# mukteshkrmishra/namazu

Hardware: AMD Instinct MI355X
Metric: schedule decisions/sec + trace-pair edit distances/sec at 1/2/4/8 MI355X (higher is better)
Workload: dtype u64; 1 GPU; configs[1] replayable seed sweep; seeds_per_gpu=1048576, events=4096, max_interval_ns=100000000, topk=64, pipeline_streams=3, parallelism=seed-range x1

## Files before the change

### include/nmz_gpu.h

```cpp
#ifndef NMZ_GPU_H
#define NMZ_GPU_H

#include <stddef.h>
#include <stdint.h>

#ifdef __cplusplus
extern "C" {
#endif

#define NMZ_ABI_VERSION 1

#define NMZ_OK 0
#define NMZ_EINVAL (-1)
#define NMZ_EHIP (-2)
#define NMZ_ENOMEM (-3)
#define NMZ_ERANGE (-4)
#define NMZ_EAGAIN (-5)

#define NMZ_EV_PRIORITIZED 0x01u
#define NMZ_EV_FAULTABLE 0x02u

#define NMZ_STAT_RNG_OVERFLOW 0x01u

#define NMZ_NONE 0xffffffffu
// ... 61 lines not shown
                         uint64_t n_seeds, const uint32_t *hint_off, const uint8_t *hint_bytes,
                         uint32_t n_events, int64_t max_interval_ns, nmz_sched_stats *stats,
                         int64_t *delays, uint64_t n_dump_seeds, uint32_t k,
                         nmz_topk_entry *topk);

typedef struct nmz_replayable_plan nmz_replayable_plan;
int nmz_replayable_plan_create(nmz_ctx *ctx, const uint32_t *hint_off, const uint8_t *hint_bytes,
                               uint32_t n_events, int64_t max_interval_ns,
                               uint64_t max_seeds, nmz_replayable_plan **out);
int nmz_replayable_plan_create_async(nmz_ctx *ctx, const uint32_t *hint_off, const uint8_t *hint_bytes,
                                     uint32_t n_events, int64_t max_interval_ns, uint64_t max_seeds,
                                     nmz_replayable_plan **out);
typedef struct nmz_replayable_seeds nmz_replayable_seeds;
int nmz_replayable_seeds_create(nmz_ctx *ctx, const uint32_t *d_seed_off, const uint8_t *d_seed_bytes,
                                uint64_t n_seeds, uint64_t dec_lo, nmz_replayable_seeds **out);
int nmz_replayable_seeds_destroy(nmz_replayable_seeds *seeds);
int nmz_replayable_sweep_seeds_topk_dev(nmz_replayable_plan *plan, const nmz_replayable_seeds *seeds, uint64_t seed0,
                                        uint32_t k, nmz_sched_stats *d_stats, nmz_topk_entry *d_topk, void *stream);
int nmz_replayable_sweep_traces(nmz_ctx *ctx, uint32_t n_traces, const uint32_t *const *hint_off,
                                const uint8_t *const *hint_bytes, const uint32_t *n_events, int64_t max_interval_ns,
                                uint64_t seed_lo, uint64_t n_seeds, uint32_t k, nmz_topk_entry *topk);
int nmz_replayable_plan_destroy(nmz_replayable_plan *plan);
int nmz_replayable_plan_kernel(const nmz_replayable_plan *plan);
int nmz_replayable_sweep_dev(nmz_replayable_plan *plan, const uint32_t *d_seed_off,
                             const uint8_t *d_seed_bytes, uint64_t n_seeds,
                             nmz_sched_stats *d_stats, void *stream);
int nmz_replayable_sweep_topk_dev(nmz_replayable_plan *plan, const uint32_t *d_seed_off,
                                  const uint8_t *d_seed_bytes, uint64_t n_seeds, uint64_t seed0,
                                  uint32_t k, nmz_sched_stats *d_stats, nmz_topk_entry *d_topk,
                                  void *stream);

int nmz_replayable_sweep_decimal_topk_dev(nmz_replayable_plan *plan, uint64_t seed_lo, uint64_t n_seeds, uint32_t k,
                                          nmz_sched_stats *d_stats, nmz_topk_entry *d_topk, void *stream);

int nmz_replayable_decide(nmz_ctx *ctx, const uint8_t *seed, uint32_t seed_len, const uint32_t *hint_off,
                          const uint8_t *hint_bytes, uint32_t n_events, int64_t max_interval_ns, int64_t *delays);

typedef struct nmz_order_constraint {
    uint32_t before;
    uint32_t after;
    int64_t margin_ns;
} nmz_order_constraint;

typedef struct nmz_order_stats {
    uint64_t sat_mask;
    int64_t min_slack_ns;
// ... 301 lines not shown
```

### namazu_amd/_lib.py

```python
import ctypes
import os
import threading

import numpy as np

HERE = os.path.dirname(os.path.abspath(__file__))
DEFAULT_LIB_PATH = os.path.join(HERE, "libnmz_gpu.so")
LIB_PATH = os.environ.get("NMZ_LIB_PATH") or DEFAULT_LIB_PATH

NMZ_OK = 0
NMZ_EINVAL = -1
NMZ_EHIP = -2
NMZ_ENOMEM = -3
NMZ_ERANGE = -4
NMZ_EAGAIN = -5

NMZ_EV_PRIORITIZED = 0x01
NMZ_EV_FAULTABLE = 0x02
NMZ_STAT_RNG_OVERFLOW = 0x01
NMZ_NONE = 0xFFFFFFFF
NMZ_ED_NCOUNTERS = 6
NMZ_ED_OPT_SINGLE_KERNEL, NMZ_ED_OPT_NO_QGRAM, NMZ_ED_OPT_COMPACT, NMZ_ED_OPT_HOST_BUILD = 1, 2, 4, 8
NMZ_ED_FP_WORDS = 8
NMZ_PROC_MILD, NMZ_PROC_EXTREME, NMZ_PROC_DIRICHLET = 0, 1, 2
# ... 61 lines not shown


_P = ctypes.c_void_p
_u64, _i64, _u32, _i32 = ctypes.c_uint64, ctypes.c_int64, ctypes.c_uint32, ctypes.c_int32
_int = ctypes.c_int
SIGNATURES = {
    "nmz_open": (_int, [_int, ctypes.POINTER(_P)]),
    "nmz_close": (_int, [_P]),
    "nmz_last_error": (ctypes.c_char_p, []),
    "nmz_abi_version": (_int, []),
    "nmz_device_count": (_int, [ctypes.POINTER(_int)]),
    "nmz_ctx_stream": (_int, [_P, ctypes.POINTER(_P)]),
    "nmz_random_params_resolve": (_int, [_i64, _i64, ctypes.c_double, _P]),
    "nmz_fnv1a64_batch": (_int, [_P, _P, _P, _u64, _P]),
    "nmz_replayable_sweep": (_int, [_P, _P, _P, _u64, _P, _P, _u32, _i64, _P, _P, _u64, _u32, _P]),
    "nmz_replayable_plan_create": (_int, [_P, _P, _P, _u32, _i64, _u64, ctypes.POINTER(_P)]),
    "nmz_replayable_plan_create_async": (_int, [_P, _P, _P, _u32, _i64, _u64, ctypes.POINTER(_P)]),
    "nmz_replayable_seeds_create": (_int, [_P, _P, _P, _u64, _u64, ctypes.POINTER(_P)]),
    "nmz_replayable_seeds_destroy": (_int, [_P]),
    "nmz_replayable_sweep_seeds_topk_dev": (_int, [_P, _P, _u64, _u32, _P, _P, _P]),
    "nmz_replayable_sweep_traces": (_int, [_P, _u32, _P, _P, _P, _i64, _u64, _u64, _u32, _P]),
    "nmz_replayable_plan_destroy": (_int, [_P]),
    "nmz_replayable_plan_kernel": (_int, [_P]),
    "nmz_replayable_sweep_dev": (_int, [_P, _P, _P, _u64, _P, _P]),
    "nmz_replayable_sweep_topk_dev": (_int, [_P, _P, _P, _u64, _u64, _u32, _P, _P, _P]),
    "nmz_replayable_order_host": (_int, [_P, _u32, _P, _P, _u32, _i64, _P, _P, _u32, _P, _P]),
    "nmz_replayable_order_plan_create": (_int, [_P, _P, _P, _u32, _i64, _P, _P, _u32, _u64, ctypes.POINTER(_P)]),
    "nmz_replayable_order_plan_destroy": (_int, [_P]),
    "nmz_replayable_order_sweep_decimal_dev": (_int, [_P, _u64, _u64, _u32, _P, _P, _P]),
    "nmz_replayable_order_sweep_dev": (_int, [_P, _P, _P, _u64, _u64, _u32, _P, _P, _P]),
    "nmz_replayable_order_sweep": (_int, [_P, _P, _P, _u64, _P, _P, _u32, _i64, _P, _P, _u32, _u32, _P, _P]),
    "nmz_replayable_order_sweep_decimal": (_int, [_P, _u64, _u64, _P, _P, _u32, _i64, _P, _P, _u32, _u32, _P, _P]),
    "nmz_replayable_decide": (_int, [_P, _P, _u32, _P, _P, _u32, _i64, _P]),
    "nmz_random_decide": (_int, [_P, _u64, _P, _P, _u32, _P, _P, _P]),
    "nmz_random_sweep": (_int, [_P, _u64, _u64, _P, _P, _u32, _P, _P, _P, _P, _u64, _u32, _P]),
    "nmz_procset_params_resolve": (_int, [ctypes.c_char_p, _int, _int, ctypes.c_double, _P]),
    "nmz_procset_decide_host": (_int, [_u64, _P, _P, _P, _u32, _P, _P, _P, _P]),
    "nmz_procset_decide": (_int, [_P, _u64, _P, _P, _P, _u32, _P, _P, _P, _P]),
    "nmz_procset_sweep": (_int, [_P, _u64, _u64, _P, _P, _P, _P, _u32, _P, _P, _P, _P, _P, _u64, _u32, _int, _P]),
    "nmz_random_plan_create": (_int, [_P, _P, _P, _u32, _P, _u64, ctypes.POINTER(_P)]),
    "nmz_random_plan_destroy": (_int, [_P]),
    "nmz_random_sweep_dev": (_int, [_P, _u64, _u64, _P, _P]),
    "nmz_ed_pairs": (_int, [_P, _P, _P, _u32, _P, _u64, _u32, _P]),
    "nmz_ed_allpairs_knn": (_int, [_P, _P, _P, _u32, _u32, _u32, _P, _P]),
    "nmz_ed_plan_create": (_int, [_P, _P, _P, _u32, _u32, ctypes.POINTER(_P)]),
    "nmz_ed_plan_destroy": (_int, [_P]),
# ... 192 lines not shown
```

### namazu_amd/csrc/replayable.hip

```cpp
#include <algorithm>
#include <cstring>
#include <cstdlib>
#include <numeric>
#include <string>
#include <vector>

#include "nmz_common.h"
#include "nmz_internal.h"
#include "replayable_plan.h"

namespace nmz {

__global__ __launch_bounds__(256) void k_replayable_table(const uint32_t *__restrict__ hoff,
                                                          const uint8_t *__restrict__ hbytes,
                                                          const uint32_t *__restrict__ perm, uint32_t E,
                                                          uint64_t m, int fast, uint4 *__restrict__ table) {
    const uint32_t pos = blockIdx.x;
    const uint32_t L = threadIdx.x;
    const uint32_t e = perm[pos];
    const uint32_t b0 = hoff[e], b1 = hoff[e + 1];
    uint64_t h = L;
    for (uint32_t i = b0; i < b1; ++i) h = fnv_step(h, hbytes[i]);
    const uint64_t C = h - (uint64_t)L * fnv_pow(b1 - b0);
    const uint32_t cm = fast ? (uint32_t)(C % m) : 0u;
// ... 454 lines not shown
int nmz_replayable_plan_create_async(nmz_ctx *ctx, const uint32_t *hint_off, const uint8_t *hint_bytes,
                                     uint32_t n_events, int64_t max_interval_ns, uint64_t max_seeds,
                                     nmz_replayable_plan **out) {
    NMZ_CHECK(ctx != nullptr, "ctx is NULL");
    CtxGuard g(ctx);
    NMZ_TRY(g.rc);
    return plan_create(ctx, hint_off, hint_bytes, n_events, max_interval_ns, max_seeds, out, true);
}

int nmz_replayable_plan_destroy(nmz_replayable_plan *plan) {
    if (!plan) return NMZ_OK;
    {
        CtxGuard g(plan->ctx);
        plan_destroy_locked(plan);
    }
    return NMZ_OK;
}

int nmz_replayable_plan_kernel(const nmz_replayable_plan *plan) {
    if (!plan) return -1;
    return plan->wt.on ? 2 : plan->oq.on ? 1 : 0;
}

int nmz_replayable_sweep_dev(nmz_replayable_plan *plan, const uint32_t *d_seed_off, const uint8_t *d_seed_bytes,
                             uint64_t n_seeds, nmz_sched_stats *d_stats, void *stream) {
    NMZ_CHECK(plan != nullptr, "plan is NULL");
    CtxGuard g(plan->ctx);
    NMZ_TRY(g.rc);
    hipStream_t st = stream ? (hipStream_t)stream : plan->ctx->stream;
    return replayable_run(plan, st, d_seed_off, d_seed_bytes, n_seeds, d_stats);
}

int nmz_replayable_sweep_topk_dev(nmz_replayable_plan *plan, const uint32_t *d_seed_off, const uint8_t *d_seed_bytes,
                                  uint64_t n_seeds, uint64_t seed0, uint32_t k, nmz_sched_stats *d_stats,
                                  nmz_topk_entry *d_topk, void *stream) {
    NMZ_CHECK(plan != nullptr, "plan is NULL");
    CtxGuard g(plan->ctx);
    NMZ_TRY(g.rc);
    hipStream_t st = stream ? (hipStream_t)stream : plan->ctx->stream;
    return replayable_run(plan, st, d_seed_off, d_seed_bytes, n_seeds, d_stats, seed0, k, d_topk);
}

int nmz_replayable_sweep_traces(nmz_ctx *ctx, uint32_t n_traces, const uint32_t *const *hint_off,
                                const uint8_t *const *hint_bytes, const uint32_t *n_events, int64_t max_interval_ns,
                                uint64_t seed_lo, uint64_t n_seeds, uint32_t k, nmz_topk_entry *topk) {
    NMZ_CHECK(ctx != nullptr, "ctx is NULL");
// ... 186 lines not shown
```

### namazu_amd/csrc/replayable_plan.h

```cpp
#pragma once
#include <array>

#include "nmz_common.h"
#include "nmz_internal.h"

namespace nmz {

struct ClassInfo {
    uint64_t pn;
    uint32_t start;
    uint32_t count;
};

constexpr uint32_t REPLAY_SEEDS_PER_UNIT_MIN = 64 * 2;
constexpr uint32_t OQ_WG = 1024;

struct SeedScratch {
    uint64_t *h0;
    Buckets b;
    uint32_t *counter;
};

inline size_t seed_scratch_bytes(uint64_t S) {
    uint64_t max_units = S / REPLAY_SEEDS_PER_UNIT_MIN + 257;
// ... 24 lines not shown
struct OqState {
    bool on = false;
    struct Pass {
        uint32_t c0, c1;
        uint64_t off16;
        uint32_t rb16;
    };
    std::vector<Pass> passes;
    uint4 *d_blob = nullptr;
    uint64_t *d_rowsum = nullptr;
    OqClass *d_classes = nullptr;
    DevBuf mem;
};
bool replay_oq_enabled();
int oq_build(OqState &o, const uint4 *d_table, uint32_t E, const ModParams &mod, const std::vector<ClassInfo> &cls,
             hipStream_t st);
int oq_sweep(const OqState &o, nmz_ctx *ctx, hipStream_t st, const Buckets &b, const uint4 *d_table, uint32_t E,
             const ModParams &mod, nmz_sched_stats *d_stats);

struct WtState {
    bool on = false;
    uint32_t rb16 = 0, n_classes = 0, msh = 0;
    uint32_t bb = 5;
    uint4 *d_blob = nullptr;
    unsigned long long *d_rowsum = nullptr;
    void *d_classes = nullptr;
    DevBuf mem;
    DevBuf aux;
};
bool wt_enabled();
struct WtClass {
    uint64_t pn;
    uint32_t start, n;
    uint32_t o_lv, o_cm;
    uint32_t o_chi, o_e;
    uint32_t o_im, o_ic;
    uint32_t K, nw;
    uint32_t rS;
    uint32_t o_mk;
    uint32_t order;
    uint32_t pad;
};
static_assert(sizeof(WtClass) == 64, "WtClass layout");

struct WtPlanHints {
    const uint32_t *hoff;
    const uint8_t *hbytes;
    const uint32_t *perm;
    uint4 *table;
    uint32_t *zero0;
    uint32_t n_zero0;
    uint32_t *zero1;
    uint32_t n_zero1;
};
bool wt_layout(WtState &w, nmz_ctx *ctx, uint32_t E, const ClassInfo *cls, uint32_t n_cls, const ModParams &mod,
               bool fused, std::vector<WtClass> &oc);
int wt_launch(WtState &w, const uint4 *d_table, uint32_t E, const ModParams &mod, hipStream_t st,
              const WtPlanHints *hints, WtClass *d_cls, unsigned long long *d_rowsum, bool sync);
int wt_build(WtState &w, nmz_ctx *ctx, const uint4 *d_table, uint32_t E, const ClassInfo *cls, uint32_t n_cls,
             const ModParams &mod, hipStream_t st);
int wt_sweep(const WtState &w, nmz_ctx *ctx, hipStream_t st, const Buckets &b, const uint4 *d_table, uint32_t E,
             const ModParams &mod, nmz_sched_stats *d_stats, uint64_t S, void *topk_scratch);
size_t wt_topk_scratch_bytes(uint64_t S);
int wt_topk(hipStream_t st, void *scratch, const uint32_t *bucket_off, const uint32_t *sorted_idx,
// ... 43 lines not shown
```

### namazu_amd/csrc/replayable_wt.hip

```cpp
#include <algorithm>
#include <cstring>
#include <numeric>
#include <cstdlib>
#include <string>
#include <vector>

#include "nmz_common.h"
#include "nmz_internal.h"
#include "replayable_plan.h"

namespace nmz {

#ifndef NMZ_WT_BRUTE
#define NMZ_WT_BRUTE 8
#endif
constexpr uint32_t WT_BRUTE = NMZ_WT_BRUTE;
constexpr uint32_t WT_NMAX = 4096;
constexpr uint32_t WT_LDS_MAX = 160 * 1024 - 256;
constexpr uint32_t WT_NONE = 0xffffffffu;
constexpr uint32_t WT_PAD = 32;
#ifdef WT_BUILD_TRACE
constexpr uint32_t WT_TRACE_PHASES = 10, WT_TRACE_WGS = 8192;
__device__ unsigned long long g_wt_build_trace[WT_TRACE_WGS * WT_TRACE_PHASES];
#define WT_STAMP(k)                                                                                              \
    do {                                                                                                         \
        if (threadIdx.x == 0 && blockIdx.y * gridDim.x + blockIdx.x < WT_TRACE_WGS)                              \
            g_wt_build_trace[(L * gridDim.x + c) * WT_TRACE_PHASES + (k)] = wall_clock64();                      \
    } while (0)
#else
#define WT_STAMP(k) \
    do {            \
    } while (0)
#endif


__host__ __device__ constexpr uint32_t wt_levels(uint32_t K, uint32_t bb) { return K > bb ? K - bb : 0; }
__host__ __device__ constexpr uint64_t wt_mask_bytes(uint32_t n, uint32_t bb) {
    return (uint64_t)((n >> bb) + 1) * ((1u << bb) + 1) * ((1u << bb) / 8);
}

template <int BB>
struct WtMask;
template <>
struct WtMask<5> {
    using T = uint32_t;
    static __device__ __forceinline__ T load(const char *mk, uint32_t i) {
        return reinterpret_cast<const uint32_t *>(mk)[i];
    }
    static __device__ __forceinline__ uint32_t count_ge(T v, uint32_t r) { return __popc(v >> r); }
    static __device__ __forceinline__ T below(T v, uint32_t r) { return __builtin_amdgcn_ubfe(v, 0u, r); }
    static __device__ __forceinline__ T low(T v, uint32_t s) { return v & (0xffffffffu >> (32u - s)); }
    static __device__ __forceinline__ T inv(T v) { return ~v; }
    static __device__ __forceinline__ bool any(T v) { return v != 0; }
    static __device__ __forceinline__ uint32_t top(T v) { return 31u - __clz(v); }
};
template <>
struct WtMask<6> {
    using T = uint64_t;
    static __device__ __forceinline__ T load(const char *mk, uint32_t i) {
        return reinterpret_cast<const uint64_t *>(mk)[i];
    }
    static __device__ __forceinline__ uint32_t count_ge(T v, uint32_t r) { return (uint32_t)__popcll(v >> r); }
// ... 323 lines not shown
    for (uint32_t i = tid; i <= n; i += WT_BT) {
        const int bm = i < n ? (int)((uint32_t)(srt[i] >> 32) >> msh) : 257;
        const int pm_ = i ? (int)((uint32_t)(srt[i - 1] >> 32) >> msh) : -1;
        for (int b = pm_ + 1; b <= min(bm, 256); ++b) im[b] = i;
        const int bc2 = i < n ? (int)(chiL[i] >> 24) : 256;
        const int pc = i ? (int)(chiL[i - 1] >> 24) : -1;
        for (int b = pc + 1; b <= min(bc2, 255); ++b) ic[b] = i;
    }
    __syncthreads();
    if (tid < 257) {
        reinterpret_cast<uint16_t *>(img + ci.o_im)[tid] = (uint16_t)im[tid];
        atomicMax(bmax + 2, (tid < 256 ? im[tid + 1] : n) - im[tid]);
    }
    if (tid < 256) {
        reinterpret_cast<uint16_t *>(img + ci.o_ic)[tid] = (uint16_t)ic[tid];
        atomicMax(bmax + 3, (tid < 255 ? ic[tid + 1] : n) - ic[tid]);
    }
    __syncthreads();
#ifndef WT_ABL_RS_ATOMIC
    if (tid == 0) atomicMax(&classes[c].rS, 32u - __clz(max(bmax[2], bmax[3])));
#endif
    WT_STAMP(5);
    WT_STAMP(6);
    const uint32_t K = ci.K, nw = ci.nw, lb = wt_levels(K, BB);
    uint2 *lv = reinterpret_cast<uint2 *>(img + ci.o_lv);
    uint16_t *cur = S0, *nxt = S0 + WT_NMAX;
    constexpr uint32_t MAXG = (WT_NMAX / 64 + 1 + WT_BW - 1) / WT_BW;
    const uint32_t ng = (nw * 32 + 63) / 64, gpw = (ng + WT_BW - 1) / WT_BW, g0 = wave * gpw;
    uint32_t *wtot = cum;
    for (uint32_t l = 0; l < lb; ++l) {
        const uint32_t h = 1u << (K - l - 1);
        uint64_t bal[MAXG];
        uint32_t vv[MAXG], tot = 0;
#pragma unroll
        for (uint32_t gi = 0; gi < MAXG; ++gi) {
            const uint32_t g = g0 + gi, j = g * 64 + lane;
            bal[gi] = 0;
            vv[gi] = 0;
            if (gi < gpw && g < ng) {
                vv[gi] = j < n ? cur[j] : 0u;
                bal[gi] = __ballot(j < n && (vv[gi] & h));
                tot += (uint32_t)__popcll(bal[gi]);
            }
        }
        if (lane == 0) wtot[wave] = tot;
        __syncthreads();
// ... 95 lines not shown
    key = k > key ? k : key;
}

#ifndef WT_SGPR_CONST
__device__ __forceinline__ uint32_t wt_v(uint32_t x) {
    uint32_t v;
    asm volatile("v_mov_b32 %0, %1" : "=v"(v) : "s"(x));
    return v;
}
#else
__device__ __forceinline__ uint32_t wt_v(uint32_t x) { return x; }
#endif

__device__ __forceinline__ uint32_t wt_ones(const uint2 *__restrict__ lvl, uint32_t s, uint32_t p) {
    const uint2 w = lvl[p >> 5];
    return w.y + __popc(w.x & ((1u << (p & 31)) - 1u)) - (s >> 1);
}


struct WtVConst {
    uint32_t st4[5];
};

template <bool BIG, int NS, int BB>
__device__ __forceinline__ void wt_seed_class(const WtVConst &vc, const WtClass &ci, const char *__restrict__ img,
                                              const uint4 *__restrict__ row, const uint64_t (&h0)[NS], uint32_t m,
                                              uint64_t mu, uint32_t m_k64, uint32_t msh, uint64_t (&sum)[NS],
                                              uint32_t (&W)[NS], uint64_t (&key)[NS]) {
    const uint32_t n = ci.n;
    uint64_t nH[NS];
    uint32_t Hm[NS], Hm2[NS];
#pragma unroll
    for (int u = 0; u < NS; ++u) {
        const uint64_t H = h0[u] * ci.pn;
        nH[u] = ~H;
        Hm[u] = BIG ? mod_barrett64(H, m, mu) : mod_barrett_small(H, m, mu);
        const uint32_t t2 = Hm[u] + m_k64;
        Hm2[u] = BIG ? ((t2 < Hm[u] || t2 >= m) ? t2 - m : t2) : min(t2, t2 - m);
    }
    if (n <= WT_BRUTE) {
#pragma unroll
        for (int u = 0; u < NS; ++u) {
            uint32_t d = 0;
            for (uint32_t i = 0; i < n; ++i) wt_decide<BIG>(row[ci.start + i], nH[u], Hm[u], Hm2[u], m, d, W[u], key[u]);
            sum[u] += (uint64_t)d * Hm[u] + (uint64_t)(n - d) * Hm2[u];
        }
        return;
// ... 37 lines not shown
        const uint32_t *ea = chi + n, *eb = cm + n;
        for (uint32_t st = (1u << rS) >> 1; st; st >>= 1) {
#pragma unroll
            for (int u = 0; u < NS; ++u) {
                const uint32_t a = *min(pa[u] + st - 1, ea), b = *min(pb[u] + st - 1, eb), c = *min(pc[u] + st - 1, eb);
                pa[u] += a < nh[u] ? st : 0u;
                pb[u] += b < XA[u] ? st : 0u;
                pc[u] += c < XB[u] ? st : 0u;
            }
        }
    }
    auto lo = [](const uint32_t *q) { return (uint32_t)reinterpret_cast<uintptr_t>(q); };
    uint32_t d[NS], RA[NS], RB[NS];
#pragma unroll
    for (int u = 0; u < NS; ++u) {
        RA[u] = (lo(pb[u]) - lo(cm)) >> 2;
        RB[u] = (lo(pc[u]) - lo(cm)) >> 2;
        d[u] = (lo(pa[u]) - lo(chi)) >> 2;
        if (chi[d[u]] == nh[u]) {
            const uint32_t nl = (uint32_t)nH[u];
            while (d[u] < n && chi[d[u]] == nh[u] && row[ci.start + d[u]].x <= nl) ++d[u];
        }
    }
    const uint2 *__restrict__ lv = reinterpret_cast<const uint2 *>(img + ci.o_lv);
    const char *__restrict__ mk = img + ci.o_mk;
    using MK = WtMask<BB>;
    using MT = typename MK::T;
    constexpr uint32_t BW = 1u << BB, BM = BW - 1;
#ifdef WT_ABL_COUNT
    const uint32_t K = ci.K, nw = ci.nw, lb = 0;
#else
    const uint32_t K = ci.K, nw = ci.nw, lb = wt_levels(K, BB);
#endif
    uint32_t oA[NS], oB[NS], cA[NS], cB[NS], lA[NS], sA[NS], qA[NS], lB[NS], sB[NS], qB[NS];
#pragma unroll
    for (int u = 0; u < NS; ++u) {
        oA[u] = oB[u] = d[u];
        cA[u] = cB[u] = 0;
        lA[u] = lB[u] = WT_NONE;
        sA[u] = qA[u] = sB[u] = qB[u] = 0;
    }
    const uint32_t nv = wt_v(n), one = wt_v(1u), five = wt_v(5u);
    if (lb) {
        const uint32_t hs = 1u << (K - 1);
#pragma unroll
        for (int u = 0; u < NS; ++u) {
            const uint2 w = lv[d[u] >> 5];
            const uint32_t o = w.y + __popc(__builtin_amdgcn_ubfe(w.x, 0u, d[u])), z = d[u] - o;
            const bool b1 = RA[u] >= hs, b2 = RB[u] >= hs;
            const bool u1 = b1 && z != 0, u2 = b2 && hs > z;
            lA[u] = u1 ? 1u : lA[u];
// ... 14 lines not shown
                const uint2 w1 = lvl[p1 >> five], w2 = lvl[p2 >> five];
                const uint32_t o1 = w1.y + __popc(__builtin_amdgcn_ubfe(w1.x, 0u, p1)) - (s1 >> one);
                const uint32_t o2 = w2.y + __popc(__builtin_amdgcn_ubfe(w2.x, 0u, p2)) - (s2 >> one);
                const uint32_t z1 = oA[u] - o1, z2 = oB[u] - o2;
                const bool b1 = RA[u] & h, b2 = RB[u] & h;
                const bool u1 = b1 && z1 != 0;
                const bool u2 = b2 && min(nv - s2, h) > z2;
                lA[u] = u1 ? l1 : lA[u];
                qA[u] = u1 ? z1 : qA[u];
                lB[u] = u2 ? l1 : lB[u];
                qB[u] = u2 ? z2 : qB[u];
                cA[u] += b1 ? 0u : o1;
                cB[u] += b2 ? 0u : o2;
                oA[u] = b1 ? o1 : z1;
                oB[u] = b2 ? o2 : z2;
            }
            h >>= 1;
            msk = (uint32_t)((int32_t)msk >> 1);
            l1 += 1;
            lvl += nw;
        }
    }
    MT belA[NS], belB[NS];
    bool hitA[NS], hitB[NS], wrapA[NS], wrapB[NS];
    uint32_t l0 = WT_NONE;
#pragma unroll
    for (int u = 0; u < NS; ++u) {
        const uint32_t bA = RA[u] & ~BM, bB = RB[u] & ~BM, rA = RA[u] & BM, rB = RB[u] & BM;
        const MT mA = MK::load(mk, bA + (bA >> BB) + oA[u]), mB = MK::load(mk, bB + (bB >> BB) + oB[u]);
        cA[u] += MK::count_ge(mA, rA);
        cB[u] += MK::count_ge(mB, rB);
        W[u] += cA[u] + (n - RB[u]) - cB[u];
        belA[u] = MK::below(mA, rA);
        belB[u] = MK::below(MK::inv(mB), rB);
        hitA[u] = MK::any(belA[u]);
        hitB[u] = MK::any(belB[u]);
        wrapA[u] = d[u] > 0 && !hitA[u] && lA[u] == WT_NONE;
        wrapB[u] = d[u] < n && !hitB[u] && lB[u] == WT_NONE;
        if (wrapA[u]) {
            lA[u] = 0;
            qA[u] = d[u];
        }
        if (wrapB[u]) {
            lB[u] = 0;
            qB[u] = d[u];
        }
        const bool dA = d[u] > 0 && !hitA[u], dB = d[u] < n && !hitB[u];
// ... 13 lines not shown
            const uint32_t h = wt_v(hs), h2 = wt_v(2 * hs), lv1 = wt_v(l);
            const uint2 *__restrict__ lvl = lv + l * nw;
#pragma unroll
            for (int u = 0; u < NS; ++u) {
                const uint32_t p1 = sA[u] + qA[u], p2 = sB[u] + qB[u];
                const uint2 w1 = lvl[p1 >> five], w2 = lvl[p2 >> five];
                const uint32_t o1 = w1.y + __popc(__builtin_amdgcn_ubfe(w1.x, 0u, p1)) - (sA[u] >> one);
                const uint32_t o2 = w2.y + __popc(__builtin_amdgcn_ubfe(w2.x, 0u, p2)) - (sB[u] >> one);
                const bool a1 = lv1 >= lA[u], a2 = lv1 >= lB[u];
                const bool g1 = a1 && o1 != 0;
                const bool g2 = a2 && min(nv - sB[u], h2) > h + o2;
                sA[u] += g1 ? h : 0u;
                qA[u] = g1 ? o1 : qA[u];
                sB[u] += g2 ? h : 0u;
                qB[u] = a2 ? (g2 ? o2 : qB[u] - o2) : qB[u];
            }
        }
    }
#pragma unroll
    for (int u = 0; u < NS; ++u) {
        const MT vA = MK::load(mk, sA[u] + (sA[u] >> BB) + qA[u]);
        const MT vB = MK::low(MK::inv(MK::load(mk, sB[u] + (sB[u] >> BB) + qB[u])), min(nv - sB[u], BW));
        const uint32_t bA = RA[u] & ~BM, bB = RB[u] & ~BM;
        const uint32_t pA = hitA[u] ? bA + MK::top(belA[u]) : sA[u] + MK::top(vA);
        const uint32_t pB = hitB[u] ? bB + MK::top(belB[u]) : sB[u] + MK::top(vB);
        if (d[u] > 0) {
            const uint32_t t = Hm[u] + cm[pA] - (wrapA[u] ? m : 0u);
            const uint64_t k = ((uint64_t)t << 32) | (0xffffffffu - ev[pA]);
            key[u] = k > key[u] ? k : key[u];
        }
        if (d[u] < n) {
            const uint32_t t = Hm2[u] + cm[pB] - (wrapB[u] ? m : 0u);
            const uint64_t k = ((uint64_t)t << 32) | (0xffffffffu - ev[pB]);
            key[u] = k > key[u] ? k : key[u];
        }
        sum[u] += (uint64_t)d[u] * Hm[u] + (uint64_t)(n - d[u]) * Hm2[u];
    }
}

constexpr uint32_t WT_CAND = 4096;
constexpr int WT_NS = 1;
struct WtChunkRec {
    unsigned long long key;
    uint32_t pos, cnt;
};
static_assert(sizeof(WtChunkRec) == 16, "WtChunkRec layout");
struct WtTopkState {
    unsigned long long cand_key[WT_CAND];
    uint32_t cand_idx[WT_CAND];
};

#ifdef WT_TRACE
__device__ unsigned long long g_wt_trace[256][16][10];
#define WT_TSTAMP(slot)                                                                                      \
    do {                                                                                                     \
        if ((threadIdx.x & 63) == 0 && blockIdx.x < 256 && (slot) < 10)                                      \
            g_wt_trace[blockIdx.x][threadIdx.x >> 6][(slot)] = wall_clock64();                               \
    } while (0)
#else
#define WT_TSTAMP(slot) \
    do {                \
    } while (0)
#endif

#ifndef WT_PRIO_TAIL
#define WT_PRIO_TAIL 0
#endif

#ifndef NMZ_WT_WAVES
#define NMZ_WT_WAVES 0
#endif
#if NMZ_WT_WAVES > 0
#define NMZ_WT_ATTR __attribute__((amdgpu_waves_per_eu(NMZ_WT_WAVES, NMZ_WT_WAVES)))
#else
#define NMZ_WT_ATTR
#endif
template <bool BIG, int NS, int BB>
__global__ __launch_bounds__(1024) NMZ_WT_ATTR void k_replayable_sweep_wt(
    const uint32_t *__restrict__ bucket_off, const uint64_t *__restrict__ sorted_h0,
    const uint32_t *__restrict__ sorted_idx, const uint4 *__restrict__ table, uint32_t E,
    const uint4 *__restrict__ blob, uint32_t rb16, const unsigned long long *__restrict__ rowsum,
    const WtClass *__restrict__ classes, uint32_t n_classes, uint32_t m, uint64_t mu, uint32_t m_k64, uint32_t msh,
    uint32_t G, nmz_sched_stats *__restrict__ stats, unsigned long long *__restrict__ span,
    WtChunkRec *__restrict__ rec) {
    constexpr uint32_t CS = 64 * NS;
    extern __shared__ uint4 wt_lds[];
    const uint32_t L = blockIdx.x / G, g = blockIdx.x % G;
    const uint32_t s0 = bucket_off[L], s1 = bucket_off[L + 1];
    const uint32_t nch = (s1 - s0 + CS - 1) / CS;
    const uint32_t c0 = g * nch / G, c1 = (g + 1) * nch / G;
    uint32_t *ctr = reinterpret_cast<uint32_t *>(wt_lds + rb16);
    if (c0 == c1) return;
    if (span && threadIdx.x == 0) atomicMax(span, ~(unsigned long long)wall_clock64());
    WT_TSTAMP(9);
    uint32_t cb = 0;
    if (rec)
        for (uint32_t t = threadIdx.x; t < L; t += blockDim.x) cb += (bucket_off[t + 1] - bucket_off[t] + CS - 1) / CS;
    {
        const uint4 *__restrict__ src = blob + (uint64_t)L * rb16;
        constexpr uint32_t B = 8;
// ... 42 lines not shown
#endif
        const uint32_t j0 = s0 + ch * CS + lane;
        uint64_t h0[NS];
        uint32_t idx[NS];
#pragma unroll
        for (int u = 0; u < NS; ++u) {
            h0[u] = h0n[u];
            idx[u] = idxn[u];
        }
        uint32_t chn = 0;
        if (lane == 0) chn = atomicAdd(ctr, 1u);
        chn = __builtin_amdgcn_readfirstlane(chn);
#pragma unroll
        for (int u = 0; u < NS; ++u) {
            const uint32_t jn = min(s0 + chn * CS + u * 64 + lane, s1 - 1);
            h0n[u] = sorted_h0[jn];
            idxn[u] = sorted_idx[jn];
        }
        uint64_t sum[NS], key[NS];
        uint32_t W[NS];
#pragma unroll
        for (int u = 0; u < NS; ++u) sum[u] = key[u] = W[u] = 0;
        for (uint32_t c = 0; c < n_classes; ++c)
            wt_seed_class<BIG, NS, BB>(vc, classes[c], img, row, h0, m, mu, m_k64, msh, sum, W, key);
        uint64_t km = 0;
#pragma unroll
        for (int u = 0; u < NS; ++u) {
            const uint32_t j = j0 + u * 64;
            const uint64_t total = sum[u] + rsum - (uint64_t)W[u] * m;
            if (j < s1) {
                const uint64_t kk = total ^ (1ull << 63);
                km = kk > km ? kk : km;
                nmz_sched_stats st;
                st.sum_delay_ns = total;
                st.max_delay_ns = (int64_t)(key[u] >> 32);
                st.argmax_event = ~(uint32_t)key[u];
                st.n_fault = 0;
                st.first_fault = NMZ_NONE;
                st.flags = 0;
                stats[idx[u]] = st;
            }
        }
        if (rec) {
            for (int o = 32; o; o >>= 1) {
                const uint64_t v = __shfl_xor(km, o, 64);
                km = v > km ? v : km;
            }
// ... 363 lines not shown
static uint32_t wt_groups() {
    static const uint32_t g = [] {
        const char *e = ab_env("NMZ_WT_G");
        const int v = e ? atoi(e) : 1;
        return (uint32_t)((v == 1 || v == 2 || v == 4 || v == 8) ? v : 1);
    }();
    return g;
}
static uint32_t wt_threads() {
    static const uint32_t t = [] {
        const char *e = ab_env("NMZ_WT_THREADS");
        const int v = e ? atoi(e) : 1024;
        return (uint32_t)((v >= 64 && v <= 1024 && v % 64 == 0) ? v : 1024);
    }();
    return t;
}

static uint32_t wt_max_bb() {
    const char *e = ab_env("NMZ_WT_BB");
    const int v = e ? atoi(e) : 6;
    return (uint32_t)((v >= 5 && v <= 7) ? v : 6);
}

constexpr size_t WT_BUILD_LDS = WT_NMAX * 8 * 2 + WT_NMAX / 2 * 4 + 2 * (WT_NMAX / 32 + 4) * 4 + 520 * 4 +
                                WT_BW * 8 + 16;

bool wt_layout(WtState &w, nmz_ctx *ctx, uint32_t E, const ClassInfo *cls, uint32_t n_cls, const ModParams &mod,
               bool fused, std::vector<WtClass> &oc) {
    w.on = false;
    if (!wt_enabled() || !mod.m32ok || E == 0 || E > 65536) return false;
    if (fused) {
        for (uint32_t c = 0; c < n_cls; ++c)
            if (cls[c].count > WT_NMAX - 1) return false;
    }
    auto r16 = [](uint64_t b) { return (b + 15) & ~15ull; };
    std::vector<ClassInfo> seg;
    for (uint32_t c = 0; c < n_cls; ++c) {
        const uint32_t n = cls[c].count, parts = (n + WT_NMAX - 2) / (WT_NMAX - 1);
        for (uint32_t k = 0, lo = 0; k < parts; ++k) {
            const uint32_t len = n / parts + (k < n % parts ? 1u : 0u);
            seg.push_back(ClassInfo{cls[c].pn, cls[c].start + lo, len});
            lo += len;
        }
    }
    n_cls = (uint32_t)seg.size();
    auto layout = [&](uint32_t bb) -> uint64_t {
    oc.assign(n_cls, WtClass{});
    uint64_t off = 0;
    for (uint32_t c = 0; c < n_cls; ++c) {
        WtClass &o = oc[c];
        o.pn = seg[c].pn;
        o.start = seg[c].start;
        o.n = seg[c].count;
        if (o.n <= WT_BRUTE) continue;
        o.K = bitlen(o.n);
        o.nw = o.n / 32 + 1;
        o.o_lv = (uint32_t)off;
        off += r16((uint64_t)wt_levels(o.K, bb) * o.nw * 8);
        o.o_cm = (uint32_t)off;
        off += r16((uint64_t)(o.n + WT_PAD) * 4);
        o.o_chi = (uint32_t)off;
        off += r16((uint64_t)(o.n + WT_PAD) * 4);
        o.o_e = (uint32_t)off;
        off += r16((uint64_t)o.n * 2);
        o.o_im = (uint32_t)off;
        off += r16(257 * 2);
        o.o_ic = (uint32_t)off;
        off += r16(256 * 2);
        o.o_mk = (uint32_t)off;
        off += r16(wt_mask_bytes(o.n, bb));
    }
    return off;
    };
    uint32_t bb = wt_max_bb();
    uint64_t off = layout(bb);
    while (bb > 5 && std::max<uint64_t>(16, r16(off)) + 32 > WT_LDS_MAX) off = layout(--bb);
    {
        std::vector<uint32_t> ord(n_cls);
        std::iota(ord.begin(), ord.end(), 0u);
        std::stable_sort(ord.begin(), ord.end(), [&](uint32_t a, uint32_t b) { return oc[a].n > oc[b].n; });
        for (uint32_t r = 0; r < n_cls; ++r) oc[r].order = ord[r];
    }
    const uint64_t rb = std::max<uint64_t>(16, r16(off));
    if (rb + 32 > WT_LDS_MAX) return false;
    if (!ctx->wt_lds_attr) {
        for (const void *f : {reinterpret_cast<const void *>(k_replayable_sweep_wt<false, 1, 5>),
                              reinterpret_cast<const void *>(k_replayable_sweep_wt<true, 1, 5>),
                              reinterpret_cast<const void *>(k_replayable_sweep_wt<false, 1, 6>),
                              reinterpret_cast<const void *>(k_replayable_sweep_wt<true, 1, 6>),
                              reinterpret_cast<const void *>(k_replayable_sweep_wt<false, 1, 7>),
                              reinterpret_cast<const void *>(k_replayable_sweep_wt<true, 1, 7>),
                              reinterpret_cast<const void *>(k_replayable_wt_build<false, 5>),
                              reinterpret_cast<const void *>(k_replayable_wt_build<true, 5>),
                              reinterpret_cast<const void *>(k_replayable_wt_build<false, 6>),
                              reinterpret_cast<const void *>(k_replayable_wt_build<true, 6>),
                              reinterpret_cast<const void *>(k_replayable_wt_build<false, 7>),
                              reinterpret_cast<const void *>(k_replayable_wt_build<true, 7>)})
            if (hipFuncSetAttribute(f, hipFuncAttributeMaxDynamicSharedMemorySize, (int)WT_LDS_MAX) != hipSuccess) {
                (void)hipGetLastError();
                return false;
            }
        ctx->wt_lds_attr = true;
    }
    w.rb16 = (uint32_t)(rb / 16);
    w.bb = bb;
    w.n_classes = n_cls;
    w.msh = mod.m32 > 255 ? bitlen(mod.m32) - 8 : 0;
    return true;
}

int wt_launch(WtState &w, const uint4 *d_table, uint32_t E, const ModParams &mod, hipStream_t st,
              const WtPlanHints *hints, WtClass *d_cls, unsigned long long *d_rowsum, bool sync) {
    NMZ_TRY(w.mem.ensure(Carve::bytes_for(256 * (size_t)w.rb16, 16)));
    w.d_blob = w.mem.as<uint4>();
    w.d_rowsum = d_rowsum;
    w.d_classes = d_cls;
    WtHints hz{};
    if (hints)
        hz = WtHints{hints->hoff, hints->hbytes, hints->perm, mod.m, mod.mu, hints->table, hints->zero0, hints->n_zero0,
                     hints->zero1, hints->n_zero1};
    auto kern = hints ? (w.bb == 7 ? k_replayable_wt_build<true, 7>
                         : w.bb == 6 ? k_replayable_wt_build<true, 6> : k_replayable_wt_build<true, 5>)
                      : (w.bb == 7 ? k_replayable_wt_build<false, 7>
                         : w.bb == 6 ? k_replayable_wt_build<false, 6> : k_replayable_wt_build<false, 5>);
    hipLaunchKernelGGL(kern, dim3(w.n_classes, 256), dim3(WT_BT), WT_BUILD_LDS, st, hints ? nullptr : d_table, E,
                       d_cls, w.msh, bitlen(mod.m32), w.d_blob, w.rb16, d_rowsum, hz);
    NMZ_HIP(hipGetLastError());
    if (sync) NMZ_HIP(hipStreamSynchronize(st));
// ... 27 lines not shown
    NMZ_CHECK(k >= 1 && k <= 64, "internal: wt_topk takes 1 <= k <= 64");
    Carve cv(scratch);
    WtTopkState *tk = cv.take<WtTopkState>(1);
    const WtChunkRec *rec = cv.take<WtChunkRec>(wt_max_chunks(S));
    hipLaunchKernelGGL(k_wt_topk_chunks<64 * WT_NS>, dim3(1), dim3(WT_SEL_THREADS), 0, st, bucket_off, rec, sorted_idx,
                       d_stats, S, seed0, k, (uint32_t)wt_max_chunks(S), tk, d_out);
    NMZ_HIP(hipGetLastError());
    return NMZ_OK;
}

int wt_sweep(const WtState &w, nmz_ctx *ctx, hipStream_t st, const Buckets &b, const uint4 *d_table, uint32_t E,
             const ModParams &mod, nmz_sched_stats *d_stats, uint64_t S, void *topk_scratch) {
    WtChunkRec *rec = nullptr;
    if (topk_scratch) {
        Carve cv(topk_scratch);
        cv.take<WtTopkState>(1);
        rec = cv.take<WtChunkRec>(wt_max_chunks(S));
    }
    const uint32_t G = wt_groups(), nt = wt_threads();
    KernelTimer kt(ctx, st, "replayable_sweep");
    unsigned long long *span = kt.span();
    const bool big = mod.m32 >= 0x80000000u;
    auto kern = big ? (w.bb == 7 ? k_replayable_sweep_wt<true, WT_NS, 7>
                       : w.bb == 6 ? k_replayable_sweep_wt<true, WT_NS, 6> : k_replayable_sweep_wt<true, WT_NS, 5>)
                    : (w.bb == 7 ? k_replayable_sweep_wt<false, WT_NS, 7>
                       : w.bb == 6 ? k_replayable_sweep_wt<false, WT_NS, 6> : k_replayable_sweep_wt<false, WT_NS, 5>);
    const size_t lds = w.rb16 * 16u + 32u;
    hipLaunchKernelGGL(kern, dim3(256 * G), dim3(nt), lds, st, b.offset, b.sorted_h0, b.sorted_idx,
                       d_table, E, w.d_blob, w.rb16, w.d_rowsum, static_cast<const WtClass *>(w.d_classes),
                       w.n_classes, mod.m32, mod.mu, mod.m_k64, w.msh, G, d_stats, span, rec);
    NMZ_HIP(hipGetLastError());
    return NMZ_OK;
}

}

#ifdef WT_TRACE
extern "C" int nmz_debug_wt_trace(unsigned long long *out) {
    return hipMemcpyFromSymbol(out, HIP_SYMBOL(nmz::g_wt_trace), sizeof(nmz::g_wt_trace)) == hipSuccess ? 0 : -1;
}
#endif

#ifdef WT_BUILD_TRACE
extern "C" int nmz_debug_wt_build_trace(unsigned long long *out, uint32_t n) {
    const uint32_t m = std::min<uint32_t>(n, nmz::WT_TRACE_WGS * nmz::WT_TRACE_PHASES);
    return hipMemcpyFromSymbol(out, HIP_SYMBOL(nmz::g_wt_build_trace), m * 8) == hipSuccess ? 0 : -1;
}
#endif
```

Baseline: 78750 billion decisions/s.

## Replace wavelet-tree levels with per-block prefix-count planes for 64-wide masks

```diff
diff --git a/include/nmz_gpu.h b/include/nmz_gpu.h
--- a/include/nmz_gpu.h
+++ b/include/nmz_gpu.h
@@ -107,6 +107,8 @@
                                 uint64_t seed_lo, uint64_t n_seeds, uint32_t k, nmz_topk_entry *topk);
 int nmz_replayable_plan_destroy(nmz_replayable_plan *plan);
 int nmz_replayable_plan_kernel(const nmz_replayable_plan *plan);
+int nmz_replayable_plan_wt_info(const nmz_replayable_plan *plan, uint32_t *bb, uint32_t *planes,
+                                uint64_t *image_bytes);
 int nmz_replayable_sweep_dev(nmz_replayable_plan *plan, const uint32_t *d_seed_off,
                              const uint8_t *d_seed_bytes, uint64_t n_seeds,
                              nmz_sched_stats *d_stats, void *stream);
diff --git a/namazu_amd/_lib.py b/namazu_amd/_lib.py
--- a/namazu_amd/_lib.py
+++ b/namazu_amd/_lib.py
@@ -107,6 +107,7 @@
     "nmz_replayable_sweep_traces": (_int, [_P, _u32, _P, _P, _P, _i64, _u64, _u64, _u32, _P]),
     "nmz_replayable_plan_destroy": (_int, [_P]),
     "nmz_replayable_plan_kernel": (_int, [_P]),
+    "nmz_replayable_plan_wt_info": (_int, [_P, ctypes.POINTER(_u32), ctypes.POINTER(_u32), ctypes.POINTER(_u64)]),
     "nmz_replayable_sweep_dev": (_int, [_P, _P, _P, _u64, _P, _P]),
     "nmz_replayable_sweep_topk_dev": (_int, [_P, _P, _P, _u64, _u64, _u32, _P, _P, _P]),
     "nmz_replayable_order_host": (_int, [_P, _u32, _P, _P, _u32, _i64, _P, _P, _u32, _P, _P]),
diff --git a/namazu_amd/csrc/replayable.hip b/namazu_amd/csrc/replayable.hip
--- a/namazu_amd/csrc/replayable.hip
+++ b/namazu_amd/csrc/replayable.hip
@@ -500,6 +500,16 @@
     return plan->wt.on ? 2 : plan->oq.on ? 1 : 0;
 }
 
+int nmz_replayable_plan_wt_info(const nmz_replayable_plan *plan, uint32_t *bb, uint32_t *planes,
+                                uint64_t *image_bytes) {
+    NMZ_CHECK(plan != nullptr, "plan is NULL");
+    NMZ_CHECK(plan->wt.on, "the plan does not run the wavelet-tree kernel");
+    if (bb) *bb = plan->wt.bb;
+    if (planes) *planes = plan->wt.planes ? 1u : 0u;
+    if (image_bytes) *image_bytes = (uint64_t)plan->wt.rb16 * 16u;
+    return NMZ_OK;
+}
+
 int nmz_replayable_sweep_dev(nmz_replayable_plan *plan, const uint32_t *d_seed_off, const uint8_t *d_seed_bytes,
                              uint64_t n_seeds, nmz_sched_stats *d_stats, void *stream) {
     NMZ_CHECK(plan != nullptr, "plan is NULL");
diff --git a/namazu_amd/csrc/replayable_plan.h b/namazu_amd/csrc/replayable_plan.h
--- a/namazu_amd/csrc/replayable_plan.h
+++ b/namazu_amd/csrc/replayable_plan.h
@@ -70,6 +70,7 @@
     bool on = false;
     uint32_t rb16 = 0, n_classes = 0, msh = 0;
     uint32_t bb = 5;
+    bool planes = false;
     uint4 *d_blob = nullptr;
     unsigned long long *d_rowsum = nullptr;
     void *d_classes = nullptr;
@@ -87,7 +88,7 @@
     uint32_t rS;
     uint32_t o_mk;
     uint32_t order;
-    uint32_t pad;
+    uint32_t o_pl;
 };
 static_assert(sizeof(WtClass) == 64, "WtClass layout");
 
diff --git a/namazu_amd/csrc/replayable_wt.hip b/namazu_amd/csrc/replayable_wt.hip
--- a/namazu_amd/csrc/replayable_wt.hip
+++ b/namazu_amd/csrc/replayable_wt.hip
@@ -38,6 +38,11 @@
 __host__ __device__ constexpr uint64_t wt_mask_bytes(uint32_t n, uint32_t bb) {
     return (uint64_t)((n >> bb) + 1) * ((1u << bb) + 1) * ((1u << bb) / 8);
 }
+
+__host__ __device__ constexpr uint64_t wt_plane_bytes(uint32_t n, uint32_t nw) {
+    return (uint64_t)((n >> 6) + 2) * nw * 8;
+}
+constexpr uint64_t WT_PLANES_MAX = 128 * 1024;
 
 template <int BB>
 struct WtMask;
@@ -407,6 +412,54 @@
 #endif
     WT_STAMP(5);
     WT_STAMP(6);
+    if constexpr (BB == 6) {
+        if (ci.o_pl) {
+            const uint32_t nbk = (n >> 6) + 1, nw = ci.nw, ng = (nw + 1) / 2;
+            uint2 *pl = reinterpret_cast<uint2 *>(img + ci.o_pl);
+            uint64_t *mk = reinterpret_cast<uint64_t *>(img + ci.o_mk);
+            uint8_t *ord = reinterpret_cast<uint8_t *>(bc) + 64 * wave;
+            const uint64_t below = (1ull << lane) - 1ull;
+            for (uint32_t b = wave; b <= nbk; b += WT_BW) {
+                uint32_t pre = 0, inb = 0, wlo = 0, whi = 0, wpre = 0;
+#pragma unroll 4
+                for (uint32_t g = 0; g < ng; ++g) {
+                    const uint32_t j = g * 64 + lane, v = j < n ? S0[j] : 0u;
+                    const uint64_t bg = __ballot(j < n && (v >> 6) >= b), be = __ballot(j < n && (v >> 6) == b);
+                    if (lane == g) {
+                        wlo = (uint32_t)bg;
+                        whi = (uint32_t)(bg >> 32);
+                        wpre = pre;
+                    }
+                    if (be >> lane & 1) ord[inb + (uint32_t)__popcll(be & below)] = (uint8_t)(v & 63);
+                    pre += (uint32_t)__popcll(bg);
+                    inb += (uint32_t)__popcll(be);
+                }
+                if (lane < ng) {
+                    pl[b * nw + 2 * lane] = make_uint2(wlo, wpre);
+                    if (2 * lane + 1 < nw) pl[b * nw + 2 * lane + 1] = make_uint2(whi, wpre + (uint32_t)__popc(wlo));
+                }
+                if (b < nbk) {
+                    __builtin_amdgcn_fence(__ATOMIC_SEQ_CST, "wavefront");
+                    __builtin_amdgcn_wave_barrier();
+                    unsigned long long v = lane < inb ? 1ull << ord[lane] : 0ull;
+                    for (int o = 1; o < 64; o <<= 1) {
+                        const unsigned long long u = __shfl_up(v, o, 64);
+                        if (lane >= (uint32_t)o) v |= u;
+                    }
+                    mk[b * 65 + lane + 1] = v;
+                    if (lane == 0) mk[b * 65] = 0;
+                    __builtin_amdgcn_fence(__ATOMIC_SEQ_CST, "wavefront");
+                    __builtin_amdgcn_wave_barrier();
+                }
+            }
+            WT_STAMP(7);
+#ifdef WT_BUILD_TRACE
+            __syncthreads();
+#endif
+            WT_STAMP(8);
+            return;
+        }
+    }
     const uint32_t K = ci.K, nw = ci.nw, lb = wt_levels(K, BB);
     uint2 *lv = reinterpret_cast<uint2 *>(img + ci.o_lv);
     uint16_t *cur = S0, *nxt = S0 + WT_NMAX;
@@ -548,7 +601,7 @@
     uint32_t st4[5];
 };
 
-template <bool BIG, int NS, int BB>
+template <bool BIG, int NS, int BB, bool PL>
 __device__ __forceinline__ void wt_seed_class(const WtVConst &vc, const WtClass &ci, const char *__restrict__ img,
                                               const uint4 *__restrict__ row, const uint64_t (&h0)[NS], uint32_t m,
                                               uint64_t mu, uint32_t m_k64, uint32_t msh, uint64_t (&sum)[NS],
@@ -632,11 +685,89 @@
             while (d[u] < n && chi[d[u]] == nh[u] && row[ci.start + d[u]].x <= nl) ++d[u];
         }
     }
-    const uint2 *__restrict__ lv = reinterpret_cast<const uint2 *>(img + ci.o_lv);
     const char *__restrict__ mk = img + ci.o_mk;
     using MK = WtMask<BB>;
     using MT = typename MK::T;
     constexpr uint32_t BW = 1u << BB, BM = BW - 1;
+    uint32_t pA[NS], pB[NS];
+    bool wrapA[NS], wrapB[NS];
+    if constexpr (PL) {
+        static_assert(!PL || BB == 6, "planes stand on 64-rank blocks");
+        const uint32_t NB = (n >> 6) + 1;
+        const uint32_t nv = wt_v(n), nw8 = wt_v(ci.nw * 8u), nbv = wt_v(NB), six = wt_v(6u);
+        const char *pd[NS];
+        auto fcount = [](const char *q, uint32_t dd) {
+            const uint2 w = *reinterpret_cast<const uint2 *>(q);
+            return w.y + __popc(__builtin_amdgcn_ubfe(w.x, 0u, dd));
+        };
+        uint32_t bA[NS], bB[NS], fA0[NS], fB0[NS], cA[NS], cB[NS];
+        MT belA[NS], belB[NS];
+        bool hitA[NS], hitB[NS];
+#pragma unroll
+        for (int u = 0; u < NS; ++u) {
+            pd[u] = img + ci.o_pl + (d[u] >> 5) * 8u;
+            bA[u] = RA[u] >> six;
+            bB[u] = RB[u] >> six;
+            const char *qa = pd[u] + bA[u] * nw8, *qb = pd[u] + bB[u] * nw8;
+            fA0[u] = fcount(qa, d[u]);
+            fB0[u] = fcount(qb, d[u]);
+            const uint32_t fA1 = fcount(qa + nw8, d[u]), fB1 = fcount(qb + nw8, d[u]);
+            const uint32_t rA = RA[u] & BM, rB = RB[u] & BM;
+            const MT mA = MK::load(mk, (RA[u] & ~BM) + bA[u] + (fA0[u] - fA1));
+            const MT mB = MK::load(mk, (RB[u] & ~BM) + bB[u] + (fB0[u] - fB1));
+            cA[u] = fA1 + MK::count_ge(mA, rA);
+            cB[u] = fB1 + MK::count_ge(mB, rB);
+            W[u] += cA[u] + (n - RB[u]) - cB[u];
+            belA[u] = MK::below(mA, rA);
+            belB[u] = MK::below(MK::inv(mB), rB);
+            hitA[u] = MK::any(belA[u]);
+            hitB[u] = MK::any(belB[u]);
+        }
+        constexpr uint32_t OFF = 0x7fffffffu;
+        uint32_t posA[NS], posB[NS], TA[NS], TB[NS], rng = 0;
+#pragma unroll
+        for (int u = 0; u < NS; ++u) {
+            const bool dA = d[u] > 0 && !hitA[u], dB = d[u] < n && !hitB[u];
+            wrapA[u] = dA && d[u] == cA[u];
+            wrapB[u] = dB && RB[u] + cB[u] == d[u];
+            posA[u] = wrapA[u] ? bA[u] : 0u;
+            posB[u] = wrapB[u] ? bB[u] : 0u;
+            TA[u] = !dA ? OFF : wrapA[u] ? 0u : fA0[u];
+            TB[u] = !dB ? OFF : wrapB[u] ? 0u : nv - (bB[u] << six) - fB0[u];
+            const uint32_t rA = !dA ? 0u : wrapA[u] ? nbv - 1u - bA[u] : bA[u] - 1u;
+            const uint32_t rB = !dB ? 0u : wrapB[u] ? nbv - 1u - bB[u] : bB[u] - 1u;
+            rng = max(rng, max(rA, rB));
+        }
+#ifdef WT_ABL_PRED
+        if (0)
+#endif
+        if (__builtin_amdgcn_ballot_w64(rng != 0)) {
+#pragma unroll
+            for (uint32_t st = 32; st; st >>= 1) {
+                if (st >= NB || !__builtin_amdgcn_ballot_w64(rng >= st)) continue;
+                const uint32_t stv = wt_v(st);
+#pragma unroll
+                for (int u = 0; u < NS; ++u) {
+                    const uint32_t qa = min(posA[u] + stv, nbv), qb = min(posB[u] + stv, nbv);
+                    const uint32_t fa = fcount(pd[u] + qa * nw8, d[u]), fb = fcount(pd[u] + qb * nw8, d[u]);
+                    posA[u] = (int32_t)fa > (int32_t)TA[u] ? qa : posA[u];
+                    posB[u] = (int32_t)(nv - (qb << six) - fb) > (int32_t)TB[u] ? qb : posB[u];
+                }
+            }
+        }
+#pragma unroll
+        for (int u = 0; u < NS; ++u) {
+            const char *qa = pd[u] + posA[u] * nw8, *qb = pd[u] + posB[u] * nw8;
+            const uint32_t oa = fcount(qa, d[u]) - fcount(qa + nw8, d[u]);
+            const uint32_t ob = fcount(qb, d[u]) - fcount(qb + nw8, d[u]);
+            const uint32_t sa = posA[u] << six, sb = posB[u] << six;
+            const MT vA = MK::load(mk, sa + posA[u] + oa);
+            const MT vB = MK::low(MK::inv(MK::load(mk, sb + posB[u] + ob)), min(nv - sb, BW));
+            pA[u] = hitA[u] ? (RA[u] & ~BM) + MK::top(belA[u]) : sa + MK::top(vA);
+            pB[u] = hitB[u] ? (RB[u] & ~BM) + MK::top(belB[u]) : sb + MK::top(vB);
+        }
+    } else {
+    const uint2 *__restrict__ lv = reinterpret_cast<const uint2 *>(img + ci.o_lv);
 #ifdef WT_ABL_COUNT
     const uint32_t K = ci.K, nw = ci.nw, lb = 0;
 #else
@@ -697,7 +828,7 @@
         }
     }
     MT belA[NS], belB[NS];
-    bool hitA[NS], hitB[NS], wrapA[NS], wrapB[NS];
+    bool hitA[NS], hitB[NS];
     uint32_t l0 = WT_NONE;
 #pragma unroll
     for (int u = 0; u < NS; ++u) {
@@ -757,16 +888,20 @@
         const MT vA = MK::load(mk, sA[u] + (sA[u] >> BB) + qA[u]);
         const MT vB = MK::low(MK::inv(MK::load(mk, sB[u] + (sB[u] >> BB) + qB[u])), min(nv - sB[u], BW));
         const uint32_t bA = RA[u] & ~BM, bB = RB[u] & ~BM;
-        const uint32_t pA = hitA[u] ? bA + MK::top(belA[u]) : sA[u] + MK::top(vA);
-        const uint32_t pB = hitB[u] ? bB + MK::top(belB[u]) : sB[u] + MK::top(vB);
+        pA[u] = hitA[u] ? bA + MK::top(belA[u]) : sA[u] + MK::top(vA);
+        pB[u] = hitB[u] ? bB + MK::top(belB[u]) : sB[u] + MK::top(vB);
+    }
+    }
+#pragma unroll
+    for (int u = 0; u < NS; ++u) {
         if (d[u] > 0) {
-            const uint32_t t = Hm[u] + cm[pA] - (wrapA[u] ? m : 0u);
-            const uint64_t k = ((uint64_t)t << 32) | (0xffffffffu - ev[pA]);
+            const uint32_t t = Hm[u] + cm[pA[u]] - (wrapA[u] ? m : 0u);
+            const uint64_t k = ((uint64_t)t << 32) | (0xffffffffu - ev[pA[u]]);
             key[u] = k > key[u] ? k : key[u];
         }
         if (d[u] < n) {
-            const uint32_t t = Hm2[u] + cm[pB] - (wrapB[u] ? m : 0u);
-            const uint64_t k = ((uint64_t)t << 32) | (0xffffffffu - ev[pB]);
+            const uint32_t t = Hm2[u] + cm[pB[u]] - (wrapB[u] ? m : 0u);
+            const uint64_t k = ((uint64_t)t << 32) | (0xffffffffu - ev[pB[u]]);
             key[u] = k > key[u] ? k : key[u];
         }
         sum[u] += (uint64_t)d[u] * Hm[u] + (uint64_t)(n - d[u]) * Hm2[u];
@@ -810,7 +945,7 @@
 #else
 #define NMZ_WT_ATTR
 #endif
-template <bool BIG, int NS, int BB>
+template <bool BIG, int NS, int BB, bool PL = false>
 __global__ __launch_bounds__(1024) NMZ_WT_ATTR void k_replayable_sweep_wt(
     const uint32_t *__restrict__ bucket_off, const uint64_t *__restrict__ sorted_h0,
     const uint32_t *__restrict__ sorted_idx, const uint4 *__restrict__ table, uint32_t E,
@@ -899,7 +1034,7 @@
 #pragma unroll
         for (int u = 0; u < NS; ++u) sum[u] = key[u] = W[u] = 0;
         for (uint32_t c = 0; c < n_classes; ++c)
-            wt_seed_class<BIG, NS, BB>(vc, classes[c], img, row, h0, m, mu, m_k64, msh, sum, W, key);
+            wt_seed_class<BIG, NS, BB, PL>(vc, classes[c], img, row, h0, m, mu, m_k64, msh, sum, W, key);
         uint64_t km = 0;
 #pragma unroll
         for (int u = 0; u < NS; ++u) {
@@ -1309,6 +1444,11 @@
     return (uint32_t)((v >= 5 && v <= 7) ? v : 6);
 }
 
+static bool wt_planes_enabled() {
+    const char *e = ab_env("NMZ_WT_PLANES");
+    return !(e && std::string(e) == "0");
+}
+
 constexpr size_t WT_BUILD_LDS = WT_NMAX * 8 * 2 + WT_NMAX / 2 * 4 + 2 * (WT_NMAX / 32 + 4) * 4 + 520 * 4 +
                                 WT_BW * 8 + 16;
 
@@ -1331,7 +1471,7 @@
         }
     }
     n_cls = (uint32_t)seg.size();
-    auto layout = [&](uint32_t bb) -> uint64_t {
+    auto layout = [&](uint32_t bb, bool planes) -> uint64_t {
     oc.assign(n_cls, WtClass{});
     uint64_t off = 0;
     for (uint32_t c = 0; c < n_cls; ++c) {
@@ -1343,7 +1483,7 @@
         o.K = bitlen(o.n);
         o.nw = o.n / 32 + 1;
         o.o_lv = (uint32_t)off;
-        off += r16((uint64_t)wt_levels(o.K, bb) * o.nw * 8);
+        off += r16(planes ? 0 : (uint64_t)wt_levels(o.K, bb) * o.nw * 8);
         o.o_cm = (uint32_t)off;
         off += r16((uint64_t)(o.n + WT_PAD) * 4);
         o.o_chi = (uint32_t)off;
@@ -1356,12 +1496,22 @@
         off += r16(256 * 2);
         o.o_mk = (uint32_t)off;
         off += r16(wt_mask_bytes(o.n, bb));
+        if (planes) {
+            o.o_pl = (uint32_t)off;
+            off += r16(wt_plane_bytes(o.n, o.nw));
+        }
     }
     return off;
     };
     uint32_t bb = wt_max_bb();
-    uint64_t off = layout(bb);
-    while (bb > 5 && std::max<uint64_t>(16, r16(off)) + 32 > WT_LDS_MAX) off = layout(--bb);
+    uint64_t off = layout(bb, false);
+    while (bb > 5 && std::max<uint64_t>(16, r16(off)) + 32 > WT_LDS_MAX) off = layout(--bb, false);
+    bool planes = false;
+    if (bb == 6 && wt_planes_enabled()) {
+        const uint64_t poff = layout(6, true);
+        planes = std::max<uint64_t>(16, r16(poff)) <= WT_PLANES_MAX;
+        off = planes ? poff : layout(6, false);
+    }
     {
         std::vector<uint32_t> ord(n_cls);
         std::iota(ord.begin(), ord.end(), 0u);
@@ -1377,6 +1527,8 @@
                               reinterpret_cast<const void *>(k_replayable_sweep_wt<true, 1, 6>),
                               reinterpret_cast<const void *>(k_replayable_sweep_wt<false, 1, 7>),
                               reinterpret_cast<const void *>(k_replayable_sweep_wt<true, 1, 7>),
+                              reinterpret_cast<const void *>(k_replayable_sweep_wt<false, 1, 6, true>),
+                              reinterpret_cast<const void *>(k_replayable_sweep_wt<true, 1, 6, true>),
                               reinterpret_cast<const void *>(k_replayable_wt_build<false, 5>),
                               reinterpret_cast<const void *>(k_replayable_wt_build<true, 5>),
                               reinterpret_cast<const void *>(k_replayable_wt_build<false, 6>),
@@ -1391,6 +1543,7 @@
     }
     w.rb16 = (uint32_t)(rb / 16);
     w.bb = bb;
+    w.planes = planes;
     w.n_classes = n_cls;
     w.msh = mod.m32 > 255 ? bitlen(mod.m32) - 8 : 0;
     return true;
@@ -1464,9 +1617,13 @@
     unsigned long long *span = kt.span();
     const bool big = mod.m32 >= 0x80000000u;
     auto kern = big ? (w.bb == 7 ? k_replayable_sweep_wt<true, WT_NS, 7>
-                       : w.bb == 6 ? k_replayable_sweep_wt<true, WT_NS, 6> : k_replayable_sweep_wt<true, WT_NS, 5>)
+                       : w.bb == 6 ? (w.planes ? k_replayable_sweep_wt<true, WT_NS, 6, true>
+                                               : k_replayable_sweep_wt<true, WT_NS, 6>)
+                                   : k_replayable_sweep_wt<true, WT_NS, 5>)
                     : (w.bb == 7 ? k_replayable_sweep_wt<false, WT_NS, 7>
-                       : w.bb == 6 ? k_replayable_sweep_wt<false, WT_NS, 6> : k_replayable_sweep_wt<false, WT_NS, 5>);
+                       : w.bb == 6 ? (w.planes ? k_replayable_sweep_wt<false, WT_NS, 6, true>
+                                               : k_replayable_sweep_wt<false, WT_NS, 6>)
+                                   : k_replayable_sweep_wt<false, WT_NS, 5>);
     const size_t lds = w.rb16 * 16u + 32u;
     hipLaunchKernelGGL(kern, dim3(256 * G), dim3(nt), lds, st, b.offset, b.sorted_h0, b.sorted_idx,
                        d_table, E, w.d_blob, w.rb16, w.d_rowsum, static_cast<const WtClass *>(w.d_classes),
```

New measurement: 85650 billion decisions/s (median of 6 runs). 1.09x the previous value.
